# hpcaitech/Open-Sora

Hardware: NVIDIA H100
Metric: denoise-steps/sec STDiT3-XL/2 64x32x32 bf16 (higher is better)
Workload: dtype bf16

## Files before the change

open-sora_b200/csrc/gemm_sm90.cu:

```cuda
#include <stdlib.h>

#include <type_traits>

#include "common.cuh"
#include "tiles.cuh"
#include "wgmma.cuh"

namespace osb {

constexpr int kBlockM = 128;
constexpr int kBlockK = 64;
constexpr int kNumThreads = 384;
constexpr int kStageBudget = 200 * 1024;
constexpr int kSmemLimit = 227 * 1024;

enum { kPlain = 0, kConv = 1, kHeadTiles = 2, kLora = 3, kText = 4, kFp8 = 5, kFp8Blk = 6, kFp8BlkLora = 7 };

struct Fp8BlockParams {
  int64_t a_ld, a_kstride;
  uint8_t* d8;
  float* d_scale;
  int64_t ldd8, ld_dscale;
  const float* col_scale;
};

struct GemmEpilogueParams {
  const __nv_bfloat16* bias;
  __nv_bfloat16* D;
  const __nv_bfloat16* R;
  const float* gate;
  const int32_t* mod_index;
  int64_t M, N, K;
  int64_t ldd, ldr;
  int64_t group_rows;
  int64_t gate_stride;
  int32_t epilogue;
};

struct HeadTileParams {
  uint8_t* base;
  int64_t kind_stride, head_stride;
  TileMap map;
  int32_t tile_bytes;
  int32_t heads, nkinds;
  uint32_t norm_mask, rope_mask;
  const __nv_bfloat16* norm_w[4];
  float eps;
  const float* cos;
  const float* sin;
};

struct ConvGeom {
  int32_t wt_log2, ht_log2;
  int32_t tiles_w, tiles_h, tiles_t, nb;
  int32_t w_out, h_out, t_out;
  int32_t sw, sh, st;
  int32_t kw_n, kh_n;
  int32_t cin_chunks;
};

__host__ __device__ constexpr bool staged_epilogue(int mode) {
  return mode == kPlain || mode == kConv || mode == kLora || mode == kFp8 || mode == kFp8Blk || mode == kFp8BlkLora;
}
__host__ __device__ constexpr bool fp8_mode(int mode) { return mode == kFp8 || mode == kFp8Blk || mode == kFp8BlkLora; }
__host__ __device__ constexpr bool lora_mode(int mode) { return mode == kLora || mode == kFp8BlkLora; }

template <int BLOCK_N, bool kStaged = false>
struct GemmCfg {
  static constexpr int A_BYTES = kBlockM * kBlockK * 2;
  static constexpr int B_BYTES = BLOCK_N * kBlockK * 2;
  static constexpr int STAGE_BYTES = A_BYTES + B_BYTES;
  static constexpr int EPI_BYTES = kStaged ? kBlockM * BLOCK_N * 2 : 0;
  static constexpr int RING_BUDGET = kStaged ? kSmemLimit - 1024 - 256 - EPI_BYTES : kStageBudget;
  static constexpr int STAGES_RAW = RING_BUDGET / STAGE_BYTES;
  static constexpr int STAGES = STAGES_RAW > 6 ? 6 : STAGES_RAW;
  static constexpr int NUM_BARS = 2 * STAGES + (kStaged ? 2 : 0);
  static constexpr int SMEM_BYTES = STAGES * STAGE_BYTES + EPI_BYTES + 1024 + 8 * NUM_BARS;
  static_assert(STAGES >= 2, "pipeline needs at least two stages");
  static_assert(SMEM_BYTES <= kSmemLimit, "shared memory");
  static_assert(B_BYTES % 1024 == 0, "W tile must keep 1024-byte swizzle-atom alignment");
  static_assert(BLOCK_N % 16 == 0 && BLOCK_N <= 256, "wgmma N");
  static_assert(!kStaged || BLOCK_N % 64 == 0, "the staged epilogue moves 64-column boxes");
};

template <int BLOCK_N, int kMode>
__global__ void __launch_bounds__(kNumThreads, 1)
gemm_bf16_kernel(const __grid_constant__ CUtensorMap tmap_a, const __grid_constant__ CUtensorMap tmap_w,
                 const GemmEpilogueParams p, const ConvGeom cg, const HeadTileParams ht,
                 const __grid_constant__ CUtensorMap tmap_u, const __grid_constant__ CUtensorMap tmap_lb,
                 const int32_t lora_k_blocks,
                 const float* a_scale, const float* w_scale,
                 const Fp8BlockParams fb,
                 const __grid_constant__ CUtensorMap tmap_r,
                 const __grid_constant__ CUtensorMap tmap_d) {
  constexpr bool kStaged = staged_epilogue(kMode);
  using Cfg = GemmCfg<BLOCK_N, kStaged>;
  constexpr int kStages = Cfg::STAGES;
  constexpr int kBK = fp8_mode(kMode) ? 2 * kBlockK : kBlockK;
  constexpr uint32_t kEpiBoxBytes = kBlockM * 128;

  extern __shared__ uint8_t smem_raw[];
  const uint32_t smem_base = (smem_u32(smem_raw) + 1023u) & ~1023u;
  const uint32_t epi_base = smem_base + kStages * Cfg::STAGE_BYTES;
  const uint32_t bar_base = epi_base + Cfg::EPI_BYTES;
  auto full_bar = [&](int s) { return bar_base + 8u * s; };
  auto empty_bar = [&](int s) { return bar_base + 8u * (kStages + s); };
  const uint32_t res_bar = bar_base + 8u * (2 * kStages);
  const uint32_t epi_free = bar_base + 8u * (2 * kStages + 1);
  auto smem_a = [&](int s) { return smem_base + s * Cfg::STAGE_BYTES; };
  auto smem_b = [&](int s) { return smem_base + s * Cfg::STAGE_BYTES + Cfg::A_BYTES; };

  const int wg = threadIdx.x >> 7;
  const int tid_wg = threadIdx.x & 127;
  const int64_t num_n_blocks = (p.N + BLOCK_N - 1) / BLOCK_N;
  const int64_t num_m_blocks =
      kMode == kConv ? (int64_t)cg.nb * cg.tiles_t * cg.tiles_h * cg.tiles_w : (p.M + kBlockM - 1) / kBlockM;
  const int64_t num_tiles = num_m_blocks * num_n_blocks;
  const int64_t num_k_blocks = (p.K + kBK - 1) / kBK;
  const int64_t total_k_blocks = lora_mode(kMode) ? num_k_blocks + lora_k_blocks : num_k_blocks;
  struct Tile {
    int64_t m_blk, n_blk;
    int n_i, t0, h0, w0;
  };
  auto tile_at = [&](int64_t t) {
    Tile tl = {t / num_n_blocks, t % num_n_blocks, 0, 0, 0, 0};
    if constexpr (kMode == kConv) {
      const int tw = (int)(tl.m_blk % cg.tiles_w);
      const int th = (int)((tl.m_blk / cg.tiles_w) % cg.tiles_h);
      const int tt = (int)((tl.m_blk / ((int64_t)cg.tiles_w * cg.tiles_h)) % cg.tiles_t);
      tl.n_i = (int)(tl.m_blk / ((int64_t)cg.tiles_w * cg.tiles_h * cg.tiles_t));
      tl.w0 = tw << cg.wt_log2;
      tl.h0 = th << cg.ht_log2;
      tl.t0 = tt * (128 >> (cg.wt_log2 + cg.ht_log2));
    }
    return tl;
  };

  if (threadIdx.x == 0) {
    tma_prefetch_desc(&tmap_a);
    tma_prefetch_desc(&tmap_w);
    if constexpr (lora_mode(kMode)) {
      tma_prefetch_desc(&tmap_u);
      tma_prefetch_desc(&tmap_lb);
    }
    if constexpr (kStaged) {
      if (p.R != nullptr) tma_prefetch_desc(&tmap_r);
      tma_prefetch_desc(&tmap_d);
      mbar_init(res_bar, 1);
      mbar_init(epi_free, 1);
    }
    for (int s = 0; s < kStages; ++s) {
      mbar_init(full_bar(s), 1);
      mbar_init(empty_bar(s), 2);
    }
    fence_barrier_init();
  }
  __syncthreads();
  pdl_wait();

  if (wg == 0) {
    asm volatile("setmaxnreg.dec.sync.aligned.u32 40;\n" ::: "memory");
    if (tid_wg == 0) {
      int stage = 0;
      uint32_t phase = 0;
      uint32_t it = 0;
      for (int64_t t = blockIdx.x; t < num_tiles; t += gridDim.x, ++it) {
        const Tile tl = tile_at(t);
        const int32_t a_row = (int32_t)(tl.m_blk * kBlockM);
        const int32_t w_row = (int32_t)(tl.n_blk * BLOCK_N);
        auto load_k_block = [&](int64_t kb) {
          mbar_wait_notrace(empty_bar(stage), phase ^ 1);
          mbar_expect_tx(full_bar(stage), Cfg::STAGE_BYTES);
          if (lora_mode(kMode) && kb >= num_k_blocks) {
            const int32_t lk0 = (int32_t)(kb - num_k_blocks) * kBlockK;
            tma_load_2d(&tmap_u, full_bar(stage), smem_a(stage), lk0, a_row);
            tma_load_2d(&tmap_lb, full_bar(stage), smem_b(stage), lk0, w_row);
          } else {
            const int32_t k0 = (int32_t)(kb * kBK);
            if constexpr (kMode == kConv) {
              const int tap = (int)(kb / cg.cin_chunks);
              const int32_t ac = (int32_t)(kb - (int64_t)tap * cg.cin_chunks) * kBlockK;
              const int32_t aw = tl.w0 * cg.sw + tap % cg.kw_n;
              const int32_t ah = tl.h0 * cg.sh + (tap / cg.kw_n) % cg.kh_n;
              const int32_t at = tl.t0 * cg.st + tap / (cg.kw_n * cg.kh_n);
              tma_load_5d(&tmap_a, full_bar(stage), smem_a(stage), ac, aw, ah, at, tl.n_i);
            } else {
              tma_load_2d(&tmap_a, full_bar(stage), smem_a(stage), k0, a_row);
            }
            tma_load_2d(&tmap_w, full_bar(stage), smem_b(stage), k0, w_row);
          }
          if (++stage == kStages) { stage = 0; phase ^= 1; }
        };
        int64_t kb = 0;
        if constexpr (kStaged) {
          if (p.R != nullptr) {
            for (; kb < min((int64_t)kStages, total_k_blocks); ++kb) load_k_block(kb);
            if (it > 0) mbar_wait_notrace(epi_free, (it - 1) & 1u);
            const int live = (int)min((int64_t)(BLOCK_N / 64), (p.N - w_row + 63) / 64);
            mbar_expect_tx(res_bar, (uint32_t)live * kEpiBoxBytes);
            for (int c = 0; c < live; ++c) {
              if constexpr (kMode == kConv)
                tma_load_5d(&tmap_r, res_bar, epi_base + c * kEpiBoxBytes, w_row + 64 * c, tl.w0, tl.h0, tl.t0, tl.n_i);
              else
                tma_load_2d(&tmap_r, res_bar, epi_base + c * kEpiBoxBytes, w_row + 64 * c, a_row);
            }
          }
        }
        for (; kb < total_k_blocks; ++kb) load_k_block(kb);
      }
      pdl_launch_dependents();
    }
    return;
  }

  asm volatile("setmaxnreg.inc.sync.aligned.u32 232;\n" ::: "memory");
  const int cw = wg - 1;
  int stage = 0;
  uint32_t phase = 0;
  uint32_t it = 0;
  auto release_epi_buffer = [&](int64_t kb) {
    if constexpr (kStaged) {
      if (kb == 0 && it > 0 && threadIdx.x == 128) {
        bulk_wait_group_read_all();
        mbar_arrive(epi_free);
      }
    }
  };
  for (int64_t t = blockIdx.x; t < num_tiles; t += gridDim.x, ++it) {
    const Tile tl = tile_at(t);
    const int64_t m_blk = tl.m_blk, n_blk = tl.n_blk;
    const int warp_in = tid_wg >> 5, lane = tid_wg & 31;
    const int r_frag = cw * 64 + warp_in * 16 + (lane >> 2);
    const int c_frag = 2 * (lane & 3);
    const float* gate_row[2] = {nullptr, nullptr};
    float sa[2] = {0.f, 0.f};
    if constexpr (kStaged && kMode != kConv) {
      const uint32_t group_rows32 = (uint32_t)(p.group_rows > 0xffffffffll ? 0xffffffffu : p.group_rows);
#pragma unroll
      for (int h = 0; h < 2; ++h) {
        const int64_t row = min(m_blk * kBlockM + r_frag + 8 * h, p.M - 1);
        if (p.epilogue == OSB_EPI_BIAS_GATE_RES && p.gate != nullptr) {
          int64_t gi = (uint32_t)row / group_rows32;
          if (p.mod_index) gi = p.mod_index[gi];
          gate_row[h] = p.gate + gi * p.gate_stride;
        }
        if constexpr (kMode == kFp8) sa[h] = __ldg(a_scale + row);
      }
    }
    float acc[BLOCK_N / 2];
#pragma unroll
    for (int i = 0; i < BLOCK_N / 2; ++i) acc[i] = 0.f;
    if constexpr (fp8_mode(kMode)) {
      float part[BLOCK_N / 2];
#pragma unroll
      for (int i = 0; i < BLOCK_N / 2; ++i) part[i] = 0.f;
      const float* sa_row0 = a_scale;
      const float* sa_row1 = a_scale;
      if constexpr (kMode != kFp8) {
        const int64_t r0 = m_blk * kBlockM + cw * 64 + (tid_wg >> 5) * 16 + ((tid_wg & 31) >> 2);
        sa_row0 = a_scale + min(r0, p.M - 1) * fb.a_ld;
        sa_row1 = a_scale + min(r0 + 8, p.M - 1) * fb.a_ld;
      }
      auto k_block = [&](int64_t kb, auto is_tail) {
        constexpr bool tail = decltype(is_tail)::value;
        float s0 = 1.f, s1 = 1.f;
        if constexpr (kMode != kFp8 && !tail) {
          s0 = __ldg(sa_row0 + kb * fb.a_kstride);
          s1 = __ldg(sa_row1 + kb * fb.a_kstride);
        }
        if constexpr (tail) {
          if (kb == num_k_blocks) {
#pragma unroll
            for (int j = 0; j < BLOCK_N / 8; ++j) {
              const int64_t n = min(n_blk * BLOCK_N + 8 * j + c_frag, p.N - 2);
              const float2 sw = __ldg(reinterpret_cast<const float2*>(w_scale + n));
              acc[4 * j] = __fmul_rn(acc[4 * j], sw.x);
              acc[4 * j + 1] = __fmul_rn(acc[4 * j + 1], sw.y);
              acc[4 * j + 2] = __fmul_rn(acc[4 * j + 2], sw.x);
              acc[4 * j + 3] = __fmul_rn(acc[4 * j + 3], sw.y);
            }
          }
        }
        mbar_wait_notrace(full_bar(stage), phase);
        const uint64_t da = make_sw128_kmajor_desc(smem_a(stage) + (uint32_t)(cw * 64 * 128));
        const uint64_t db = make_sw128_kmajor_desc(smem_b(stage));
        wgmma_fence_regs(part);
        wgmma_fence();
#pragma unroll
        for (int k = 0; k < 4; ++k) {
          if constexpr (tail)
            Wgmma<BLOCK_N>::mma(part, da + (uint64_t)(2 * k), db + (uint64_t)(2 * k), k > 0 ? 1u : 0u);
          else
            WgmmaFp8<BLOCK_N>::mma(part, da + (uint64_t)(2 * k), db + (uint64_t)(2 * k), k > 0 ? 1u : 0u);
        }
        wgmma_commit();
        release_epi_buffer(kb);
        wgmma_wait<0>();
        wgmma_fence_regs(part);
        if (tid_wg == 0) mbar_arrive(empty_bar(stage));
        if constexpr (kMode != kFp8) {
#pragma unroll
          for (int j = 0; j < BLOCK_N / 8; ++j) {
            acc[4 * j] = fmaf(part[4 * j], s0, acc[4 * j]);
            acc[4 * j + 1] = fmaf(part[4 * j + 1], s0, acc[4 * j + 1]);
            acc[4 * j + 2] = fmaf(part[4 * j + 2], s1, acc[4 * j + 2]);
            acc[4 * j + 3] = fmaf(part[4 * j + 3], s1, acc[4 * j + 3]);
          }
        } else {
#pragma unroll
          for (int i = 0; i < BLOCK_N / 2; ++i) acc[i] += part[i];
        }
        if (++stage == kStages) { stage = 0; phase ^= 1; }
      };
      for (int64_t kb = 0; kb < num_k_blocks; ++kb) k_block(kb, std::false_type{});
      if constexpr (kMode == kFp8BlkLora) {
        for (int64_t kb = num_k_blocks; kb < total_k_blocks; ++kb) k_block(kb, std::true_type{});
      }
    } else {
      int prev = 0;
      for (int64_t kb = 0; kb < total_k_blocks; ++kb) {
        mbar_wait_notrace(full_bar(stage), phase);
        const uint64_t da = make_sw128_kmajor_desc(smem_a(stage) + (uint32_t)(cw * 64 * 128));
        const uint64_t db = make_sw128_kmajor_desc(smem_b(stage));
        wgmma_fence_regs(acc);
        wgmma_fence();
#pragma unroll
        for (int k = 0; k < kBlockK / 16; ++k)
          Wgmma<BLOCK_N>::mma(acc, da + (uint64_t)(2 * k), db + (uint64_t)(2 * k), (kb > 0 || k > 0) ? 1u : 0u);
        wgmma_commit();
        release_epi_buffer(kb);
        wgmma_wait<1>();
        wgmma_fence_regs(acc);
        if (kb > 0 && tid_wg == 0) mbar_arrive(empty_bar(prev));
        prev = stage;
        if (++stage == kStages) { stage = 0; phase ^= 1; }
      }
      wgmma_wait<0>();
      wgmma_fence_regs(acc);
      if (tid_wg == 0) mbar_arrive(empty_bar(prev));
    }

    if constexpr (lora_mode(kMode)) {
      const float* col_scale = kMode == kLora ? w_scale : fb.col_scale;
      if (col_scale != nullptr) {
#pragma unroll
        for (int j = 0; j < BLOCK_N / 8; ++j) {
          const int64_t n = min(n_blk * BLOCK_N + 8 * j + c_frag, p.N - 2);
          const float2 cs = __ldg(reinterpret_cast<const float2*>(col_scale + n));
          acc[4 * j] *= cs.x;
          acc[4 * j + 1] *= cs.y;
          acc[4 * j + 2] *= cs.x;
          acc[4 * j + 3] *= cs.y;
        }
      }
    }

    if constexpr ((kMode == kFp8Blk || kMode == kFp8BlkLora) && BLOCK_N == 128) {
      if (p.epilogue == OSB_EPI_BIAS_GELU_TANH_FP8) {
        const int64_t n0 = n_blk * BLOCK_N + c_frag;
#pragma unroll
        for (int h = 0; h < 2; ++h) {
          const int64_t row = m_blk * kBlockM + r_frag + 8 * h;
          float amax = 0.f;
#pragma unroll
          for (int j = 0; j < BLOCK_N / 8; ++j) {
            const int64_t n = n0 + 8 * j;
            float v0 = acc[4 * j + 2 * h], v1 = acc[4 * j + 2 * h + 1];
            if constexpr (kMode == kFp8Blk) {
              const float2 sw = __ldg(reinterpret_cast<const float2*>(w_scale + n));
              v0 *= sw.x;
              v1 *= sw.y;
            }
            if (p.bias) {
              const float2 b = unpack_bf16x2(__ldg(reinterpret_cast<const uint32_t*>(p.bias + n)));
              v0 += b.x;
              v1 += b.y;
            }
            v0 = gelu_tanh(v0);
            v1 = gelu_tanh(v1);
            acc[4 * j + 2 * h] = v0;
            acc[4 * j + 2 * h + 1] = v1;
            amax = fmaxf(amax, fmaxf(fabsf(v0), fabsf(v1)));
          }
          amax = fmaxf(amax, __shfl_xor_sync(0xffffffffu, amax, 1));
          amax = fmaxf(amax, __shfl_xor_sync(0xffffffffu, amax, 2));
          const float s = amax > 0.f ? amax / 448.0f : 1.0f;
          if (row < p.M) {
            uint8_t* drow = fb.d8 + row * fb.ldd8;
#pragma unroll
            for (int j = 0; j < BLOCK_N / 8; ++j)
              *reinterpret_cast<uint16_t*>(drow + n0 + 8 * j) =
                  (uint16_t)e4m3x2(acc[4 * j + 2 * h] / s, acc[4 * j + 2 * h + 1] / s);
            if (c_frag == 0) fb.d_scale[row * fb.ld_dscale + n_blk] = s;
          }
        }
        continue;
      }
    }

    if constexpr (kMode == kHeadTiles) {
      constexpr int D = BLOCK_N / 2;
      using HT = HeadTileCfg<D>;
      constexpr int JH = D / 8;
      const int C = ht.heads * D;
      const uint32_t chunk_bytes = (uint32_t)ht.map.TR * 128u;
#pragma unroll
      for (int h = 0; h < 2; ++h) {
        const int64_t row = m_blk * kBlockM + r_frag + 8 * h;
        const bool row_ok = row < p.M;
        uint32_t pos = 0, tile_i = 0;
        int r = 0;
        if (row_ok) tile_of_row(ht.map, (uint32_t)row, tile_i, pos, r);
#pragma unroll
        for (int hh = 0; hh < 2; ++hh) {
          const int64_t col0 = n_blk * BLOCK_N + hh * D;
          if (col0 >= p.N) continue;
          const int kidx = (int)((uint32_t)col0 / (uint32_t)C);
          const int head = (int)((uint32_t)col0 - (uint32_t)kidx * (uint32_t)C) / D;
          const int kind = kidx % ht.nkinds;
          float x[JH][2];
#pragma unroll
          for (int j = 0; j < JH; ++j) {
            x[j][0] = acc[4 * (hh * JH + j) + 2 * h];
            x[j][1] = acc[4 * (hh * JH + j) + 2 * h + 1];
            if (p.bias) {
              const float2 b = unpack_bf16x2(__ldg(reinterpret_cast<const uint32_t*>(p.bias + col0 + 8 * j + c_frag)));
              x[j][0] += b.x;
              x[j][1] += b.y;
            }
          }
          if ((ht.norm_mask >> kind) & 1u) {
            float ss = 0.f;
#pragma unroll
            for (int j = 0; j < JH; ++j) ss += x[j][0] * x[j][0] + x[j][1] * x[j][1];
            ss += __shfl_xor_sync(0xffffffffu, ss, 1);
            ss += __shfl_xor_sync(0xffffffffu, ss, 2);
            const float rs = rsqrtf(ss * (1.0f / D) + ht.eps);
            const __nv_bfloat16* w = kind == 0 ? ht.norm_w[0] : (kind == 1 ? ht.norm_w[1] : (kind == 2 ? ht.norm_w[2] : ht.norm_w[3]));
#pragma unroll
            for (int j = 0; j < JH; ++j) {
              const float2 f = unpack_bf16x2(__ldg(reinterpret_cast<const uint32_t*>(w + 8 * j + c_frag)));
              x[j][0] *= rs * f.x;
              x[j][1] *= rs * f.y;
            }
          }
          if ((ht.rope_mask >> kind) & 1u) {
#pragma unroll
            for (int j = 0; j < JH; ++j) {
              const int64_t i = (int64_t)pos * (D / 2) + (8 * j + c_frag) / 2;
              const float cc = __ldg(ht.cos + i), sn = __ldg(ht.sin + i);
              const float a = x[j][0], b = x[j][1];
              x[j][0] = a * cc - b * sn;
              x[j][1] = b * cc + a * sn;
            }
          }
          uint8_t* dst = ht.base + (int64_t)kidx * ht.kind_stride + (int64_t)head * ht.head_stride + (int64_t)tile_i * ht.tile_bytes;
          const bool odd = (lane & 1) != 0, high = (lane & 2) != 0;
#pragma unroll
          for (int j0 = 0; j0 < HT::MAIN * 8; j0 += 4) {
            uint32_t u0 = pack_bf16x2(x[j0][0], x[j0][1]), u1 = pack_bf16x2(x[j0 + 1][0], x[j0 + 1][1]);
            uint32_t u2 = pack_bf16x2(x[j0 + 2][0], x[j0 + 2][1]), u3 = pack_bf16x2(x[j0 + 3][0], x[j0 + 3][1]);
            uint32_t s0 = __shfl_xor_sync(0xffffffffu, odd ? u0 : u1, 1);
            uint32_t s1 = __shfl_xor_sync(0xffffffffu, odd ? u2 : u3, 1);
            if (odd) { u0 = s0; u2 = s1; } else { u1 = s0; u3 = s1; }
            s0 = __shfl_xor_sync(0xffffffffu, high ? u0 : u2, 2);
            s1 = __shfl_xor_sync(0xffffffffu, high ? u1 : u3, 2);
            if (high) { u0 = s0; u1 = s1; } else { u2 = s0; u3 = s1; }
            if (row_ok)
              *reinterpret_cast<uint4*>(dst + tile_unit_off<HT::MAIN>(r, j0 + (lane & 3), chunk_bytes)) = make_uint4(u0, u1, u2, u3);
          }
          if (!row_ok) continue;
#pragma unroll
          for (int j = HT::MAIN * 8; j < JH; ++j)
            *reinterpret_cast<uint32_t*>(dst + tile_unit_off<HT::MAIN>(r, j, chunk_bytes) + c_frag * 2) = pack_bf16x2(x[j][0], x[j][1]);
          if constexpr (HT::UP > HT::U)
            *reinterpret_cast<uint32_t*>(dst + tile_unit_off<HT::MAIN>(r, HT::U, chunk_bytes) + c_frag * 2) = 0u;
        }
      }
    } else if constexpr (kMode == kText) {
#pragma unroll
      for (int h = 0; h < 2; ++h) {
        const int64_t row = m_blk * kBlockM + r_frag + 8 * h;
        if (row >= p.M) continue;
        __nv_bfloat16* drow = p.D + row * p.ldd;
#pragma unroll
        for (int j = 0; j < BLOCK_N / 8; ++j) {
          const int64_t n = n_blk * BLOCK_N + 8 * j + c_frag;
          if (n >= p.N) continue;
          float v0 = acc[4 * j + 2 * h], v1 = acc[4 * j + 2 * h + 1];
          if (p.bias) {
            const float2 b = unpack_bf16x2(__ldg(reinterpret_cast<const uint32_t*>(p.bias + n)));
            v0 += b.x;
            v1 += b.y;
          }
          if (p.epilogue == OSB_EPI_GATED_GELU) {
            drow[n >> 1] = __float2bfloat16_rn(gelu_tanh(v0) * v1);
          } else {
            v0 = v0 / (1.0f + __expf(-1.702f * v0));
            v1 = v1 / (1.0f + __expf(-1.702f * v1));
            *reinterpret_cast<uint32_t*>(drow + n) = pack_bf16x2(v0, v1);
          }
        }
      }
    } else {
      static_assert(kStaged, "every other mode has its own epilogue");
      uint8_t* const epi = smem_raw + (epi_base - smem_u32(smem_raw));
      const bool gate_res = p.epilogue == OSB_EPI_BIAS_GATE_RES;
      if (!gate_res) gate_row[0] = gate_row[1] = nullptr;
      const bool has_res = gate_res && p.R != nullptr;
      if (p.R != nullptr)
        mbar_wait_notrace(res_bar, it & 1u);
      else if (it > 0)
        mbar_wait_notrace(epi_free, (it - 1) & 1u);
      auto body = [&](auto gelu) {
#pragma unroll
        for (int j = 0; j < BLOCK_N / 8; ++j) {
          const int64_t n = min(n_blk * BLOCK_N + 8 * j + c_frag, p.N - 2);
          float2 sw = make_float2(1.f, 1.f), b = make_float2(-0.f, -0.f);
          if constexpr (kMode == kFp8 || kMode == kFp8Blk) sw = __ldg(reinterpret_cast<const float2*>(w_scale + n));
          if (p.bias) b = unpack_bf16x2(__ldg(reinterpret_cast<const uint32_t*>(p.bias + n)));
#pragma unroll
          for (int h = 0; h < 2; ++h) {
            const int li = r_frag + 8 * h;
            uint32_t* const cell = reinterpret_cast<uint32_t*>(epi + (j >> 3) * kEpiBoxBytes + li * 128 +
                                                               (((j & 7) ^ (li & 7)) << 4) + c_frag * 2);
            float v0 = acc[4 * j + 2 * h], v1 = acc[4 * j + 2 * h + 1];
            if constexpr (kMode == kFp8) {
              v0 = __fmul_rn(v0, __fmul_rn(sa[h], sw.x));
              v1 = __fmul_rn(v1, __fmul_rn(sa[h], sw.y));
            } else if constexpr (kMode == kFp8Blk) {
              v0 = __fmul_rn(v0, sw.x);
              v1 = __fmul_rn(v1, sw.y);
            }
            v0 = __fadd_rn(v0, b.x);
            v1 = __fadd_rn(v1, b.y);
            if constexpr (decltype(gelu)::value) {
              v0 = gelu_tanh(v0);
              v1 = gelu_tanh(v1);
            } else {
              const float2 g = gate_row[h] ? __ldg(reinterpret_cast<const float2*>(gate_row[h] + n)) : make_float2(1.f, 1.f);
              const float2 rv = has_res ? unpack_bf16x2(*cell) : make_float2(-0.f, -0.f);
              v0 = __fadd_rn(__fmul_rn(v0, g.x), rv.x);
              v1 = __fadd_rn(__fmul_rn(v1, g.y), rv.y);
            }
            *cell = pack_bf16x2(v0, v1);
          }
        }
      };
      if (p.epilogue == OSB_EPI_BIAS_GELU_TANH)
        body(std::true_type{});
      else
        body(std::false_type{});
      fence_proxy_async_smem();
      named_barrier_sync(1, 256);
      if (threadIdx.x == 128) {
        const int32_t n0 = (int32_t)(n_blk * BLOCK_N);
        const int live = (int)min((int64_t)(BLOCK_N / 64), (p.N - n0 + 63) / 64);
        for (int c = 0; c < live; ++c) {
          if constexpr (kMode == kConv)
            tma_store_5d(&tmap_d, epi_base + c * kEpiBoxBytes, n0 + 64 * c, tl.w0, tl.h0, tl.t0, tl.n_i);
          else
            tma_store_2d(&tmap_d, epi_base + c * kEpiBoxBytes, n0 + 64 * c, (int32_t)(m_blk * kBlockM));
        }
        bulk_commit_group();
      }
    }
  }
  if constexpr (kStaged) {
    if (threadIdx.x == 128) bulk_wait_group_read_all();
  }
}

template <int BLOCK_N, int kMode>
static int launch_kernel(const CUtensorMap& ta, const CUtensorMap& tw, const GemmEpilogueParams& p, const ConvGeom& cg,
                         const HeadTileParams& ht, int64_t tiles, cudaStream_t stream, const CUtensorMap* tu = nullptr,
                         const CUtensorMap* tlb = nullptr, int32_t lora_k_blocks = 0, const float* a_scale = nullptr,
                         const float* w_scale = nullptr, const Fp8BlockParams& fb = Fp8BlockParams{},
                         const CUtensorMap* tr = nullptr, const CUtensorMap* td = nullptr) {
  if (tiles >= (1ll << 31)) { set_error("osb gemm: too many output tiles (%lld)", (long long)tiles); return OSB_ERR_UNSUPPORTED; }
  const int64_t grid = tiles < sm_count() ? tiles : sm_count();
  cudaLaunchAttribute attr[2];
  cudaLaunchConfig_t cfg = launch_config(dim3((unsigned)grid), dim3(kNumThreads),
                                         GemmCfg<BLOCK_N, staged_epilogue(kMode)>::SMEM_BYTES, stream, attr);
  OSB_CHECK_CUDA(cudaLaunchKernelEx(&cfg, gemm_bf16_kernel<BLOCK_N, kMode>, ta, tw, p, cg, ht, tu ? *tu : ta,
                                    tlb ? *tlb : tw, lora_k_blocks, a_scale, w_scale, fb, tr ? *tr : ta, td ? *td : ta));
  count_launch();
  return OSB_OK;
}

static int make_epilogue_maps(const GemmEpilogueParams& p, CUtensorMap* tr, CUtensorMap* td) {
  if (int rc = make_tmap_2d_bf16(td, p.D, p.M, p.N, p.ldd, kBlockM, 64)) return rc;
  if (p.R != nullptr) return make_tmap_2d_bf16(tr, p.R, p.M, p.N, p.ldr, kBlockM, 64);
  *tr = *td;
  return OSB_OK;
}

template <int D>
static int launch_gemm_ht(const osb_gemm_args& a, const HeadTileParams& ht, cudaStream_t stream) {
  constexpr int BLOCK_N = 2 * D;
  CUtensorMap ta, tw;
  int rc = make_tmap_2d_bf16(&ta, a.A, a.M, a.K, a.lda, kBlockM, kBlockK);
  if (rc) return rc;
  rc = make_tmap_2d_bf16(&tw, a.W, a.N, a.K, a.ldw, BLOCK_N, kBlockK);
  if (rc) return rc;
  GemmEpilogueParams p = {};
  p.bias = static_cast<const __nv_bfloat16*>(a.bias);
  p.M = a.M; p.N = a.N; p.K = a.K;
  p.group_rows = a.M;
  p.epilogue = OSB_EPI_BIAS;
  const int64_t tiles = ((a.M + kBlockM - 1) / kBlockM) * ((a.N + BLOCK_N - 1) / BLOCK_N);
  ConvGeom cg = {};
  return launch_kernel<BLOCK_N, kHeadTiles>(ta, tw, p, cg, ht, tiles, stream);
}

template <int BLOCK_N>
static int launch_gemm(const osb_gemm_args& a, bool has_res, cudaStream_t stream, const osb_lora_args* lora = nullptr) {
  CUtensorMap ta, tw;
  int rc = make_tmap_2d_bf16(&ta, a.A, a.M, a.K, a.lda, kBlockM, kBlockK);
  if (rc) return rc;
  rc = make_tmap_2d_bf16(&tw, a.W, a.N, a.K, a.ldw, BLOCK_N, kBlockK);
  if (rc) return rc;
  GemmEpilogueParams p = {};
  p.bias = static_cast<const __nv_bfloat16*>(a.bias);
  p.D = static_cast<__nv_bfloat16*>(a.D);
  p.R = has_res ? static_cast<const __nv_bfloat16*>(a.R) : nullptr;
  p.gate = a.gate;
  p.mod_index = a.mod_index;
  p.M = a.M; p.N = a.N; p.K = a.K;
  p.ldd = a.ldd;
  p.ldr = a.ldr;
  p.group_rows = a.group_rows > 0 ? a.group_rows : a.M;
  p.gate_stride = a.gate_stride;
  p.epilogue = a.epilogue;
  const int64_t tiles = ((a.M + kBlockM - 1) / kBlockM) * ((a.N + BLOCK_N - 1) / BLOCK_N);
  ConvGeom cg = {};
  HeadTileParams ht = {};
  if (lora == nullptr && a.epilogue >= OSB_EPI_GATED_GELU) return launch_kernel<BLOCK_N, kText>(ta, tw, p, cg, ht, tiles, stream);
  CUtensorMap tr, td;
  if ((rc = make_epilogue_maps(p, &tr, &td))) return rc;
  if (lora == nullptr)
    return launch_kernel<BLOCK_N, kPlain>(ta, tw, p, cg, ht, tiles, stream, nullptr, nullptr, 0, nullptr, nullptr,
                                          Fp8BlockParams{}, &tr, &td);
  CUtensorMap tu, tlb;
  if ((rc = make_tmap_2d_bf16(&tu, lora->U, a.M, lora->r, lora->ldu, kBlockM, kBlockK))) return rc;
  if ((rc = make_tmap_2d_bf16(&tlb, lora->B, a.N, lora->r, lora->ldb, BLOCK_N, kBlockK))) return rc;
  return launch_kernel<BLOCK_N, kLora>(ta, tw, p, cg, ht, tiles, stream, &tu, &tlb, (lora->r + kBlockK - 1) / kBlockK,
                                       nullptr, lora->col_scale, Fp8BlockParams{}, &tr, &td);
}

template <int BLOCK_N, int kMode>
static int init_one() {
  OSB_CHECK_CUDA(cudaFuncSetAttribute(gemm_bf16_kernel<BLOCK_N, kMode>, cudaFuncAttributeMaxDynamicSharedMemorySize,
                                      GemmCfg<BLOCK_N, staged_epilogue(kMode)>::SMEM_BYTES));
  return OSB_OK;
}

int gemm_init() {
  int rc = 0;
  if ((rc = init_one<128, kHeadTiles>())) return rc;
  if ((rc = init_one<144, kHeadTiles>())) return rc;
  if ((rc = init_one<256, kHeadTiles>())) return rc;
  if ((rc = init_one<64, kPlain>())) return rc;
  if ((rc = init_one<128, kPlain>())) return rc;
  if ((rc = init_one<192, kPlain>())) return rc;
  if ((rc = init_one<256, kPlain>())) return rc;
  if ((rc = init_one<64, kConv>())) return rc;
  if ((rc = init_one<128, kConv>())) return rc;
  if ((rc = init_one<192, kConv>())) return rc;
  if ((rc = init_one<256, kConv>())) return rc;
  if ((rc = init_one<64, kLora>())) return rc;
  if ((rc = init_one<128, kLora>())) return rc;
  if ((rc = init_one<192, kLora>())) return rc;
  if ((rc = init_one<256, kLora>())) return rc;
  if ((rc = init_one<64, kText>())) return rc;
  if ((rc = init_one<128, kText>())) return rc;
  if ((rc = init_one<192, kText>())) return rc;
  if ((rc = init_one<256, kText>())) return rc;
  if ((rc = init_one<64, kFp8>())) return rc;
  if ((rc = init_one<128, kFp8>())) return rc;
  if ((rc = init_one<64, kFp8Blk>())) return rc;
  if ((rc = init_one<128, kFp8Blk>())) return rc;
  if ((rc = init_one<64, kFp8BlkLora>())) return rc;
  if ((rc = init_one<128, kFp8BlkLora>())) return rc;
  return OSB_OK;
}

static int pick_block_n(int64_t M, int64_t N) {
  if (N <= 64) return 64;
  const int cands[3] = {256, 192, 128};
  int best = 256;
  int64_t best_cost = INT64_MAX;
  for (int i = 0; i < 3; ++i) {
    const int bn = cands[i];
    const int64_t tiles = ((M + kBlockM - 1) / kBlockM) * ((N + bn - 1) / bn);
    const int64_t waves = (tiles + sm_count() - 1) / sm_count();
    const int64_t cost = waves * (bn + 16);
    if (cost < best_cost) { best_cost = cost; best = bn; }
  }
  return best;
}

template <int BLOCK_N, int kMode = kFp8>
static int launch_gemm_fp8(const osb_gemm_fp8_args& a, cudaStream_t stream, const Fp8BlockParams& fb = Fp8BlockParams{},
                           const osb_lora_args* lora = nullptr) {
  CUtensorMap ta, tw;
  int rc = make_tmap_2d_e4m3(&ta, a.A, a.M, a.K, a.lda, kBlockM, 2 * kBlockK);
  if (rc) return rc;
  rc = make_tmap_2d_e4m3(&tw, a.W, a.N, a.K, a.ldw, BLOCK_N, 2 * kBlockK);
  if (rc) return rc;
  GemmEpilogueParams p = {};
  p.bias = static_cast<const __nv_bfloat16*>(a.bias);
  p.D = static_cast<__nv_bfloat16*>(a.D);
  p.R = a.epilogue == OSB_EPI_BIAS_GATE_RES ? static_cast<const __nv_bfloat16*>(a.R) : nullptr;
  p.gate = a.gate;
  p.mod_index = a.mod_index;
  p.M = a.M; p.N = a.N; p.K = a.K;
  p.ldd = a.ldd;
  p.ldr = a.ldr;
  p.group_rows = a.group_rows > 0 ? a.group_rows : a.M;
  p.gate_stride = a.gate_stride;
  p.epilogue = a.epilogue;
  const int64_t tiles = ((a.M + kBlockM - 1) / kBlockM) * ((a.N + BLOCK_N - 1) / BLOCK_N);
  ConvGeom cg = {};
  HeadTileParams ht = {};
  CUtensorMap tr = ta, td = ta;
  if (a.epilogue != OSB_EPI_BIAS_GELU_TANH_FP8 && (rc = make_epilogue_maps(p, &tr, &td))) return rc;
  if constexpr (kMode == kFp8BlkLora) {
    CUtensorMap tu, tlb;
    if ((rc = make_tmap_2d_bf16(&tu, lora->U, a.M, lora->r, lora->ldu, kBlockM, kBlockK))) return rc;
    if ((rc = make_tmap_2d_bf16(&tlb, lora->B, a.N, lora->r, lora->ldb, BLOCK_N, kBlockK))) return rc;
    return launch_kernel<BLOCK_N, kMode>(ta, tw, p, cg, ht, tiles, stream, &tu, &tlb, (lora->r + kBlockK - 1) / kBlockK,
                                         a.a_scale, a.w_scale, fb, &tr, &td);
  }
  return launch_kernel<BLOCK_N, kMode>(ta, tw, p, cg, ht, tiles, stream, nullptr, nullptr, 0, a.a_scale, a.w_scale, fb,
                                       &tr, &td);
}

template <int BLOCK_N>
static int launch_conv(const osb_conv3d_args& a, const ConvGeom& cg, const uint32_t box[5], cudaStream_t stream) {
  CUtensorMap ta, tw;
  const uint64_t cp = a.cp;
  const uint64_t dims[5] = {a.narrow ? 64 : cp, (uint64_t)a.wp, (uint64_t)a.hp, (uint64_t)a.tp, (uint64_t)a.nb};
  const uint64_t str[4] = {cp * 2, (uint64_t)a.wp * cp * 2, (uint64_t)a.hp * a.wp * cp * 2,
                           (uint64_t)a.tp * a.hp * a.wp * cp * 2};
  const uint32_t es[5] = {1, (uint32_t)a.sw, (uint32_t)a.sh, (uint32_t)a.st, 1};
  int rc = make_tmap_5d_bf16(&ta, a.x_pad, dims, str, box, es);
  if (rc) return rc;
  const int64_t K = (int64_t)(a.narrow ? a.kt * a.kh : a.kt * a.kh * a.kw * (a.cp / 64)) * 64;
  rc = make_tmap_2d_bf16(&tw, a.w, a.cout, K, K, BLOCK_N, kBlockK);
  if (rc) return rc;
  GemmEpilogueParams p = {};
  p.bias = static_cast<const __nv_bfloat16*>(a.bias);
  p.D = static_cast<__nv_bfloat16*>(a.y);
  p.R = static_cast<const __nv_bfloat16*>(a.residual);
  p.M = (int64_t)a.nb * a.t_out * a.h_out * a.w_out;
  p.N = a.cout;
  p.K = K;
  p.ldd = a.cout;
  p.ldr = a.cout;
  p.group_rows = p.M;
  p.epilogue = a.residual ? OSB_EPI_BIAS_GATE_RES : OSB_EPI_BIAS;
  const int64_t tiles = (int64_t)cg.nb * cg.tiles_t * cg.tiles_h * cg.tiles_w * ((a.cout + BLOCK_N - 1) / BLOCK_N);
  HeadTileParams ht = {};
  const uint64_t cout = (uint64_t)a.cout;
  const uint64_t odims[5] = {cout, (uint64_t)a.w_out, (uint64_t)a.h_out, (uint64_t)a.t_out, (uint64_t)a.nb};
  const uint64_t ostr[4] = {cout * 2, (uint64_t)a.w_out * cout * 2, (uint64_t)a.h_out * a.w_out * cout * 2,
                            (uint64_t)a.t_out * a.h_out * a.w_out * cout * 2};
  const uint32_t obox[5] = {64, 1u << cg.wt_log2, 1u << cg.ht_log2, 128u >> (cg.wt_log2 + cg.ht_log2), 1};
  const uint32_t ones[5] = {1, 1, 1, 1, 1};
  CUtensorMap tr, td;
  if ((rc = make_tmap_5d_bf16(&td, a.y, odims, ostr, obox, ones))) return rc;
  tr = td;
  if (a.residual && (rc = make_tmap_5d_bf16(&tr, a.residual, odims, ostr, obox, ones))) return rc;
  return launch_kernel<BLOCK_N, kConv>(ta, tw, p, cg, ht, tiles, stream, nullptr, nullptr, 0, nullptr, nullptr,
                                       Fp8BlockParams{}, &tr, &td);
}

}

namespace osb {

static int check_lora_args(const char* fn, const osb_lora_args& l) {
  OSB_REQUIRE(l.U && l.B, "%s: null U or B", fn);
  OSB_REQUIRE(l.r > 0 && l.r % 8 == 0, "%s: rank r must be a positive multiple of 8 (zero-pad A and B), got %d", fn, l.r);
  OSB_REQUIRE(l.ldu >= l.r && l.ldb >= l.r && l.ldu % 8 == 0 && l.ldb % 8 == 0 &&
              ((reinterpret_cast<uintptr_t>(l.U) | reinterpret_cast<uintptr_t>(l.B)) & 15) == 0,
              "%s: U and B must be 16-byte aligned with ldu, ldb >= r and multiples of 8 (r %d ldu %lld ldb %lld)", fn,
              l.r, (long long)l.ldu, (long long)l.ldb);
  OSB_REQUIRE((reinterpret_cast<uintptr_t>(l.col_scale) & 7) == 0, "%s: col_scale must be 8-byte aligned", fn);
  return OSB_OK;
}

static int gemm_dispatch(const char* fn, const osb_gemm_args* args, const osb_lora_args* lora, void* stream) {
  if (!initialised()) { set_error("osb_init() has not been called"); return OSB_ERR_NOT_INIT; }
  OSB_REQUIRE(args != nullptr, "%s: null args", fn);
  const osb_gemm_args& a = *args;
  OSB_REQUIRE(a.A && a.W && a.D, "%s: null operand", fn);
  OSB_REQUIRE(a.M > 0 && a.N > 0 && a.K > 0, "%s: empty problem (M %lld N %lld K %lld)", fn,
              (long long)a.M, (long long)a.N, (long long)a.K);
  OSB_REQUIRE(a.K % 8 == 0 && a.N % 8 == 0, "%s: K and N must be multiples of 8 (K %lld N %lld)", fn,
              (long long)a.K, (long long)a.N);
  OSB_REQUIRE(a.ldd % 8 == 0 && (reinterpret_cast<uintptr_t>(a.D) & 15) == 0,
              "%s: D must be 16-byte aligned with ldd %% 8 == 0", fn);
  OSB_REQUIRE(a.epilogue >= OSB_EPI_BIAS && a.epilogue <= OSB_EPI_BIAS_QUICK_GELU,
              "%s: unknown epilogue %d", fn, a.epilogue);
  OSB_REQUIRE(lora == nullptr || a.epilogue <= OSB_EPI_BIAS_GATE_RES,
// ... 250 lines not shown
```

Measured before the change: 12.00.

## Add ping-pong consumer warpgroup scheduling for narrow plain and head-tile GEMMs

For plain and head-tile GEMMs with BLOCK_N<=144, each consumer warpgroup now owns a whole 128-row tile on alternating tiles instead of splitting rows. Turn barriers serialize their mainloops so one warpgroup's epilogue overlaps the other's MMA. A second epilogue buffer is added per warpgroup, which reduces pipeline stages to fit shared memory and doubles accumulator registers per thread.

```diff
diff --git a/open-sora_b200/csrc/gemm_sm90.cu b/open-sora_b200/csrc/gemm_sm90.cu
--- a/open-sora_b200/csrc/gemm_sm90.cu
+++ b/open-sora_b200/csrc/gemm_sm90.cu
@@ -64,20 +64,27 @@
 }
 __host__ __device__ constexpr bool fp8_mode(int mode) { return mode == kFp8 || mode == kFp8Blk || mode == kFp8BlkLora; }
 __host__ __device__ constexpr bool lora_mode(int mode) { return mode == kLora || mode == kFp8BlkLora; }
-
-template <int BLOCK_N, bool kStaged = false>
+__host__ __device__ constexpr bool pingpong(int mode, int block_n) {
+  return (mode == kPlain || mode == kHeadTiles) && block_n <= 144;
+}
+
+template <int BLOCK_N, int kMode>
 struct GemmCfg {
+  static constexpr bool kStaged = staged_epilogue(kMode);
+  static constexpr bool kPingPong = pingpong(kMode, BLOCK_N);
   static constexpr int A_BYTES = kBlockM * kBlockK * 2;
   static constexpr int B_BYTES = BLOCK_N * kBlockK * 2;
   static constexpr int STAGE_BYTES = A_BYTES + B_BYTES;
-  static constexpr int EPI_BYTES = kStaged ? kBlockM * BLOCK_N * 2 : 0;
+  static constexpr int EPI_TILE_BYTES = kStaged ? kBlockM * BLOCK_N * 2 : 0;
+  static constexpr int EPI_BYTES = (kPingPong ? 2 : 1) * EPI_TILE_BYTES;
   static constexpr int RING_BUDGET = kStaged ? kSmemLimit - 1024 - 256 - EPI_BYTES : kStageBudget;
   static constexpr int STAGES_RAW = RING_BUDGET / STAGE_BYTES;
   static constexpr int STAGES = STAGES_RAW > 6 ? 6 : STAGES_RAW;
-  static constexpr int NUM_BARS = 2 * STAGES + (kStaged ? 2 : 0);
+  static constexpr int NUM_BARS = 2 * STAGES + (kStaged ? (kPingPong ? 4 : 2) : 0) + (kPingPong ? 2 : 0);
   static constexpr int SMEM_BYTES = STAGES * STAGE_BYTES + EPI_BYTES + 1024 + 8 * NUM_BARS;
   static_assert(STAGES >= 2, "pipeline needs at least two stages");
   static_assert(SMEM_BYTES <= kSmemLimit, "shared memory");
+  static_assert(!kPingPong || !kStaged || BLOCK_N != 128 || STAGES == 5, "ping-pong 128: two 32 KB buffers + 5 stages");
   static_assert(B_BYTES % 1024 == 0, "W tile must keep 1024-byte swizzle-atom alignment");
   static_assert(BLOCK_N % 16 == 0 && BLOCK_N <= 256, "wgmma N");
   static_assert(!kStaged || BLOCK_N % 64 == 0, "the staged epilogue moves 64-column boxes");
@@ -93,20 +100,23 @@
                  const Fp8BlockParams fb,
                  const __grid_constant__ CUtensorMap tmap_r,
                  const __grid_constant__ CUtensorMap tmap_d) {
-  constexpr bool kStaged = staged_epilogue(kMode);
-  using Cfg = GemmCfg<BLOCK_N, kStaged>;
+  using Cfg = GemmCfg<BLOCK_N, kMode>;
+  constexpr bool kStaged = Cfg::kStaged;
+  constexpr bool kPingPong = Cfg::kPingPong;
+  constexpr int kHalves = kPingPong ? 2 : 1;
   constexpr int kStages = Cfg::STAGES;
   constexpr int kBK = fp8_mode(kMode) ? 2 * kBlockK : kBlockK;
   constexpr uint32_t kEpiBoxBytes = kBlockM * 128;
 
   extern __shared__ uint8_t smem_raw[];
   const uint32_t smem_base = (smem_u32(smem_raw) + 1023u) & ~1023u;
-  const uint32_t epi_base = smem_base + kStages * Cfg::STAGE_BYTES;
-  const uint32_t bar_base = epi_base + Cfg::EPI_BYTES;
+  auto epi_base = [&](int c) { return smem_base + kStages * Cfg::STAGE_BYTES + c * Cfg::EPI_TILE_BYTES; };
+  const uint32_t bar_base = smem_base + kStages * Cfg::STAGE_BYTES + Cfg::EPI_BYTES;
   auto full_bar = [&](int s) { return bar_base + 8u * s; };
   auto empty_bar = [&](int s) { return bar_base + 8u * (kStages + s); };
-  const uint32_t res_bar = bar_base + 8u * (2 * kStages);
-  const uint32_t epi_free = bar_base + 8u * (2 * kStages + 1);
+  auto res_bar = [&](int c) { return bar_base + 8u * (2 * kStages + 2 * c); };
+  auto epi_free = [&](int c) { return bar_base + 8u * (2 * kStages + 2 * c + 1); };
+  auto turn_bar = [&](int c) { return bar_base + 8u * (2 * kStages + (kStaged ? 4 : 0) + c); };
   auto smem_a = [&](int s) { return smem_base + s * Cfg::STAGE_BYTES; };
   auto smem_b = [&](int s) { return smem_base + s * Cfg::STAGE_BYTES + Cfg::A_BYTES; };
 
@@ -146,12 +156,18 @@
     if constexpr (kStaged) {
       if (p.R != nullptr) tma_prefetch_desc(&tmap_r);
       tma_prefetch_desc(&tmap_d);
-      mbar_init(res_bar, 1);
-      mbar_init(epi_free, 1);
+      for (int c = 0; c < kHalves; ++c) {
+        mbar_init(res_bar(c), 1);
+        mbar_init(epi_free(c), 1);
+      }
+    }
+    if constexpr (kPingPong) {
+      mbar_init(turn_bar(0), 1);
+      mbar_init(turn_bar(1), 1);
     }
     for (int s = 0; s < kStages; ++s) {
       mbar_init(full_bar(s), 1);
-      mbar_init(empty_bar(s), 2);
+      mbar_init(empty_bar(s), kPingPong ? 1 : 2);
     }
     fence_barrier_init();
   }
@@ -194,15 +210,18 @@
         int64_t kb = 0;
         if constexpr (kStaged) {
           if (p.R != nullptr) {
+            const int buf = kPingPong ? (int)(it & 1u) : 0;
+            const uint32_t own_it = kPingPong ? it >> 1 : it;
             for (; kb < min((int64_t)kStages, total_k_blocks); ++kb) load_k_block(kb);
-            if (it > 0) mbar_wait_notrace(epi_free, (it - 1) & 1u);
+            if (own_it > 0) mbar_wait_notrace(epi_free(buf), (own_it - 1) & 1u);
             const int live = (int)min((int64_t)(BLOCK_N / 64), (p.N - w_row + 63) / 64);
-            mbar_expect_tx(res_bar, (uint32_t)live * kEpiBoxBytes);
+            mbar_expect_tx(res_bar(buf), (uint32_t)live * kEpiBoxBytes);
             for (int c = 0; c < live; ++c) {
+              const uint32_t box = epi_base(buf) + c * kEpiBoxBytes;
               if constexpr (kMode == kConv)
-                tma_load_5d(&tmap_r, res_bar, epi_base + c * kEpiBoxBytes, w_row + 64 * c, tl.w0, tl.h0, tl.t0, tl.n_i);
+                tma_load_5d(&tmap_r, res_bar(buf), box, w_row + 64 * c, tl.w0, tl.h0, tl.t0, tl.n_i);
               else
-                tma_load_2d(&tmap_r, res_bar, epi_base + c * kEpiBoxBytes, w_row + 64 * c, a_row);
+                tma_load_2d(&tmap_r, res_bar(buf), box, w_row + 64 * c, a_row);
             }
           }
         }
@@ -215,41 +234,60 @@
 
   asm volatile("setmaxnreg.inc.sync.aligned.u32 232;\n" ::: "memory");
   const int cw = wg - 1;
+  const int buf = kPingPong ? cw : 0;
+  const bool store_thread = kPingPong ? tid_wg == 0 : threadIdx.x == 128;
   int stage = 0;
   uint32_t phase = 0;
-  uint32_t it = 0;
+  auto skip_tile = [&]() {
+    const int64_t s = stage + total_k_blocks;
+    stage = (int)(s % kStages);
+    phase ^= (uint32_t)(s / kStages) & 1u;
+  };
+  if (kPingPong && cw == 1) skip_tile();
+  uint32_t it = kPingPong ? cw : 0;
+  auto own_it = [&]() { return kPingPong ? it >> 1 : it; };
   auto release_epi_buffer = [&](int64_t kb) {
     if constexpr (kStaged) {
-      if (kb == 0 && it > 0 && threadIdx.x == 128) {
+      if (kb == 0 && own_it() > 0 && store_thread) {
         bulk_wait_group_read_all();
-        mbar_arrive(epi_free);
+        mbar_arrive(epi_free(buf));
       }
     }
   };
-  for (int64_t t = blockIdx.x; t < num_tiles; t += gridDim.x, ++it) {
-    const Tile tl = tile_at(t);
-    const int64_t m_blk = tl.m_blk, n_blk = tl.n_blk;
+  for (;; it += kPingPong ? 2 : 1) {
+    const int64_t t = blockIdx.x + (int64_t)it * gridDim.x;
+    if (t >= num_tiles) break;
+    Tile tl = {};
+    if constexpr (!kPingPong) tl = tile_at(t);
+    const int64_t& m_blk = tl.m_blk;
+    const int64_t& n_blk = tl.n_blk;
     const int warp_in = tid_wg >> 5, lane = tid_wg & 31;
-    const int r_frag = cw * 64 + warp_in * 16 + (lane >> 2);
+    const int r_frag = (kPingPong ? 0 : cw * 64) + warp_in * 16 + (lane >> 2);
     const int c_frag = 2 * (lane & 3);
     const float* gate_row[2] = {nullptr, nullptr};
     float sa[2] = {0.f, 0.f};
-    if constexpr (kStaged && kMode != kConv) {
-      const uint32_t group_rows32 = (uint32_t)(p.group_rows > 0xffffffffll ? 0xffffffffu : p.group_rows);
-#pragma unroll
-      for (int h = 0; h < 2; ++h) {
-        const int64_t row = min(m_blk * kBlockM + r_frag + 8 * h, p.M - 1);
-        if (p.epilogue == OSB_EPI_BIAS_GATE_RES && p.gate != nullptr) {
-          int64_t gi = (uint32_t)row / group_rows32;
-          if (p.mod_index) gi = p.mod_index[gi];
-          gate_row[h] = p.gate + gi * p.gate_stride;
-        }
-        if constexpr (kMode == kFp8) sa[h] = __ldg(a_scale + row);
-      }
-    }
-    float acc[BLOCK_N / 2];
-#pragma unroll
-    for (int i = 0; i < BLOCK_N / 2; ++i) acc[i] = 0.f;
+    auto row_operands = [&](int mh) {
+      if constexpr (kStaged && kMode != kConv) {
+        const uint32_t group_rows32 = (uint32_t)(p.group_rows > 0xffffffffll ? 0xffffffffu : p.group_rows);
+#pragma unroll
+        for (int h = 0; h < 2; ++h) {
+          const int64_t row = min(m_blk * kBlockM + r_frag + 64 * mh + 8 * h, p.M - 1);
+          if (p.epilogue == OSB_EPI_BIAS_GATE_RES && p.gate != nullptr) {
+            int64_t gi = (uint32_t)row / group_rows32;
+            if (p.mod_index) gi = p.mod_index[gi];
+            gate_row[h] = p.gate + gi * p.gate_stride;
+          }
+          if constexpr (kMode == kFp8) sa[h] = __ldg(a_scale + row);
+        }
+      }
+    };
+    if constexpr (!kPingPong) row_operands(0);
+    float accs[kHalves][BLOCK_N / 2];
+    float (&acc)[BLOCK_N / 2] = accs[0];
+#pragma unroll
+    for (int mh = 0; mh < kHalves; ++mh)
+#pragma unroll
+      for (int i = 0; i < BLOCK_N / 2; ++i) accs[mh][i] = 0.f;
     if constexpr (fp8_mode(kMode)) {
       float part[BLOCK_N / 2];
 #pragma unroll
@@ -317,27 +355,47 @@
         for (int64_t kb = num_k_blocks; kb < total_k_blocks; ++kb) k_block(kb, std::true_type{});
       }
     } else {
+      if constexpr (kPingPong) {
+        if (it > 0) mbar_wait_notrace(turn_bar(cw), ((it - 1) >> 1) & 1u);
+      }
       int prev = 0;
       for (int64_t kb = 0; kb < total_k_blocks; ++kb) {
         mbar_wait_notrace(full_bar(stage), phase);
-        const uint64_t da = make_sw128_kmajor_desc(smem_a(stage) + (uint32_t)(cw * 64 * 128));
+        const uint64_t da = make_sw128_kmajor_desc(smem_a(stage) + (uint32_t)((kPingPong ? 0 : cw) * 64 * 128));
+        const uint64_t da1 = make_sw128_kmajor_desc(smem_a(stage) + (uint32_t)(64 * 128));
         const uint64_t db = make_sw128_kmajor_desc(smem_b(stage));
-        wgmma_fence_regs(acc);
+#pragma unroll
+        for (int mh = 0; mh < kHalves; ++mh) wgmma_fence_regs(accs[mh]);
         wgmma_fence();
 #pragma unroll
-        for (int k = 0; k < kBlockK / 16; ++k)
-          Wgmma<BLOCK_N>::mma(acc, da + (uint64_t)(2 * k), db + (uint64_t)(2 * k), (kb > 0 || k > 0) ? 1u : 0u);
+        for (int k = 0; k < kBlockK / 16; ++k) {
+          if constexpr (kPingPong) {
+            Wgmma<BLOCK_N>::mma(accs[0], da + (uint64_t)(2 * k), db + (uint64_t)(2 * k), (kb > 0 || k > 0) ? 1u : 0u);
+            Wgmma<BLOCK_N>::mma(accs[1], da1 + (uint64_t)(2 * k), db + (uint64_t)(2 * k), (kb > 0 || k > 0) ? 1u : 0u);
+          } else {
+            Wgmma<BLOCK_N>::mma(acc, da + (uint64_t)(2 * k), db + (uint64_t)(2 * k), (kb > 0 || k > 0) ? 1u : 0u);
+          }
+        }
         wgmma_commit();
+        if constexpr (kPingPong) {
+          if (kb == total_k_blocks - 1 && tid_wg == 0) mbar_arrive(turn_bar(cw ^ 1));
+        }
         release_epi_buffer(kb);
         wgmma_wait<1>();
-        wgmma_fence_regs(acc);
+#pragma unroll
+        for (int mh = 0; mh < kHalves; ++mh) wgmma_fence_regs(accs[mh]);
         if (kb > 0 && tid_wg == 0) mbar_arrive(empty_bar(prev));
         prev = stage;
         if (++stage == kStages) { stage = 0; phase ^= 1; }
       }
       wgmma_wait<0>();
-      wgmma_fence_regs(acc);
+#pragma unroll
+      for (int mh = 0; mh < kHalves; ++mh) wgmma_fence_regs(accs[mh]);
       if (tid_wg == 0) mbar_arrive(empty_bar(prev));
+      if constexpr (kPingPong) {
+        skip_tile();
+        tl = tile_at(t);
+      }
     }
 
     if constexpr (lora_mode(kMode)) {
@@ -405,8 +463,9 @@
       const int C = ht.heads * D;
       const uint32_t chunk_bytes = (uint32_t)ht.map.TR * 128u;
 #pragma unroll
-      for (int h = 0; h < 2; ++h) {
-        const int64_t row = m_blk * kBlockM + r_frag + 8 * h;
+      for (int i = 0; i < 2 * kHalves; ++i) {
+        const int mh = i >> 1, h = i & 1;
+        const int64_t row = m_blk * kBlockM + r_frag + 64 * mh + 8 * h;
         const bool row_ok = row < p.M;
         uint32_t pos = 0, tile_i = 0;
         int r = 0;
@@ -421,8 +480,8 @@
           float x[JH][2];
 #pragma unroll
           for (int j = 0; j < JH; ++j) {
-            x[j][0] = acc[4 * (hh * JH + j) + 2 * h];
-            x[j][1] = acc[4 * (hh * JH + j) + 2 * h + 1];
+            x[j][0] = accs[mh][4 * (hh * JH + j) + 2 * h];
+            x[j][1] = accs[mh][4 * (hh * JH + j) + 2 * h + 1];
             if (p.bias) {
               const float2 b = unpack_bf16x2(__ldg(reinterpret_cast<const uint32_t*>(p.bias + col0 + 8 * j + c_frag)));
               x[j][0] += b.x;
@@ -504,24 +563,32 @@
       }
     } else {
       static_assert(kStaged, "every other mode has its own epilogue");
-      uint8_t* const epi = smem_raw + (epi_base - smem_u32(smem_raw));
+      uint8_t* const epi = smem_raw + (epi_base(buf) - smem_u32(smem_raw));
       const bool gate_res = p.epilogue == OSB_EPI_BIAS_GATE_RES;
       if (!gate_res) gate_row[0] = gate_row[1] = nullptr;
       const bool has_res = gate_res && p.R != nullptr;
       if (p.R != nullptr)
-        mbar_wait_notrace(res_bar, it & 1u);
-      else if (it > 0)
-        mbar_wait_notrace(epi_free, (it - 1) & 1u);
+        mbar_wait_notrace(res_bar(buf), own_it() & 1u);
+      else if (own_it() > 0)
+        mbar_wait_notrace(epi_free(buf), (own_it() - 1) & 1u);
       auto body = [&](auto gelu) {
+#pragma unroll 1
+        for (int mh = 0; mh < kHalves; ++mh) {
+          const __nv_bfloat16* bias = p.bias;
+          asm volatile("" : "+l"(bias));
+          if constexpr (kPingPong) row_operands(mh);
 #pragma unroll
         for (int j = 0; j < BLOCK_N / 8; ++j) {
+          if constexpr (kPingPong) {
+            if ((j & 7) == 0) asm volatile("" ::: "memory");
+          }
           const int64_t n = min(n_blk * BLOCK_N + 8 * j + c_frag, p.N - 2);
           float2 sw = make_float2(1.f, 1.f), b = make_float2(-0.f, -0.f);
           if constexpr (kMode == kFp8 || kMode == kFp8Blk) sw = __ldg(reinterpret_cast<const float2*>(w_scale + n));
-          if (p.bias) b = unpack_bf16x2(__ldg(reinterpret_cast<const uint32_t*>(p.bias + n)));
+          if (bias) b = unpack_bf16x2(__ldg(reinterpret_cast<const uint32_t*>(bias + n)));
 #pragma unroll
           for (int h = 0; h < 2; ++h) {
-            const int li = r_frag + 8 * h;
+            const int li = r_frag + 64 * mh + 8 * h;
             uint32_t* const cell = reinterpret_cast<uint32_t*>(epi + (j >> 3) * kEpiBoxBytes + li * 128 +
                                                                (((j & 7) ^ (li & 7)) << 4) + c_frag * 2);
             float v0 = acc[4 * j + 2 * h], v1 = acc[4 * j + 2 * h + 1];
@@ -546,28 +613,36 @@
             *cell = pack_bf16x2(v0, v1);
           }
         }
+        if constexpr (kPingPong) {
+#pragma unroll
+          for (int i = 0; i < BLOCK_N / 2; ++i) acc[i] = accs[1][i];
+        }
+        }
       };
       if (p.epilogue == OSB_EPI_BIAS_GELU_TANH)
         body(std::true_type{});
       else
         body(std::false_type{});
       fence_proxy_async_smem();
-      named_barrier_sync(1, 256);
-      if (threadIdx.x == 128) {
+      if (kPingPong && buf == 1)
+        named_barrier_sync(2, 128);
+      else
+        named_barrier_sync(1, kPingPong ? 128 : 256);
+      if (store_thread) {
         const int32_t n0 = (int32_t)(n_blk * BLOCK_N);
         const int live = (int)min((int64_t)(BLOCK_N / 64), (p.N - n0 + 63) / 64);
         for (int c = 0; c < live; ++c) {
           if constexpr (kMode == kConv)
-            tma_store_5d(&tmap_d, epi_base + c * kEpiBoxBytes, n0 + 64 * c, tl.w0, tl.h0, tl.t0, tl.n_i);
+            tma_store_5d(&tmap_d, epi_base(buf) + c * kEpiBoxBytes, n0 + 64 * c, tl.w0, tl.h0, tl.t0, tl.n_i);
           else
-            tma_store_2d(&tmap_d, epi_base + c * kEpiBoxBytes, n0 + 64 * c, (int32_t)(m_blk * kBlockM));
+            tma_store_2d(&tmap_d, epi_base(buf) + c * kEpiBoxBytes, n0 + 64 * c, (int32_t)(m_blk * kBlockM));
         }
         bulk_commit_group();
       }
     }
   }
   if constexpr (kStaged) {
-    if (threadIdx.x == 128) bulk_wait_group_read_all();
+    if (store_thread) bulk_wait_group_read_all();
   }
 }
 
@@ -581,7 +656,7 @@
   const int64_t grid = tiles < sm_count() ? tiles : sm_count();
   cudaLaunchAttribute attr[2];
   cudaLaunchConfig_t cfg = launch_config(dim3((unsigned)grid), dim3(kNumThreads),
-                                         GemmCfg<BLOCK_N, staged_epilogue(kMode)>::SMEM_BYTES, stream, attr);
+                                         GemmCfg<BLOCK_N, kMode>::SMEM_BYTES, stream, attr);
   OSB_CHECK_CUDA(cudaLaunchKernelEx(&cfg, gemm_bf16_kernel<BLOCK_N, kMode>, ta, tw, p, cg, ht, tu ? *tu : ta,
                                     tlb ? *tlb : tw, lora_k_blocks, a_scale, w_scale, fb, tr ? *tr : ta, td ? *td : ta));
   count_launch();
@@ -651,7 +726,7 @@
 template <int BLOCK_N, int kMode>
 static int init_one() {
   OSB_CHECK_CUDA(cudaFuncSetAttribute(gemm_bf16_kernel<BLOCK_N, kMode>, cudaFuncAttributeMaxDynamicSharedMemorySize,
-                                      GemmCfg<BLOCK_N, staged_epilogue(kMode)>::SMEM_BYTES));
+                                      GemmCfg<BLOCK_N, kMode>::SMEM_BYTES));
   return OSB_OK;
 }
 
```

Result: no change. 12.08, median of 6 (+0.6%).
